# alibaba/TorchEasyRec

Hardware: NVIDIA H100
Metric: samples/sec (DLRM-Criteo synth, train step fwd+bwd+optimizer) (higher is better)
Workload: dtype f32

## Files before the change

### torcheasyrec_b200/csrc/tzk_interact_wide.cu

```cuda
#include <stdint.h>
#include <stdio.h>
#include <stdlib.h>

#ifdef TZK_CPU_SHIM
#include "cuda_cpu_shim.h"
#include "sm90_cpu_emu.h"
#include "sm90_wgmma_emu.h"
typedef void* tzk_stream_t;
#define TZK_REQUIRE(cond, ...) do { if (!(cond)) return 1; } while (0)
#define TZK_CHECK_LAUNCH(name) do {} while (0)
#else
#include <cuda.h>
#include "tzk_common.cuh"
#define TZK_DYN_SMEM(type, name) extern __shared__ __align__(1024) type name[]
#include "tzk_launch.cuh"
#endif

namespace {
#ifndef TZK_CPU_SHIM
#include "tzk_sm90_ptx.h"
#endif
#include "tzk_tma.h"
#include "tzk_wgmma.cuh"
namespace tzk_itc {
__device__ __forceinline__ uint32_t cvt_tf32(float x) { return tf32_bits(x); }
__device__ __forceinline__ void mma_tf32(float (&c)[4], const uint32_t (&a)[4], const uint32_t (&b)[2]) { ::mma_tf32(c, a, b); }
}
#include "tzk_interact_tc.cuh"

__device__ __forceinline__ float4 load_l2(const float* p) {
#ifdef TZK_CPU_SHIM
  return *reinterpret_cast<const float4*>(p);
#else
  return __ldcg(reinterpret_cast<const float4*>(p));
#endif
}

constexpr int FB_M = 64;
constexpr int FB_THREADS = 512;
constexpr int FB_WARPS = FB_THREADS / 32;
constexpr int FB_CHUNKS = (tzk_itc::kRow + 31) / 32;
constexpr int FB_PAIR_CHUNKS = tzk_itc::kInter / 32;
constexpr int FB_BOX = 32 * 128;
constexpr int FB_STAGE = 4 * FB_BOX;
constexpr int FB_STAGES = 3;
constexpr int FB_LDP = 360;
constexpr int FB_P_OFF = FB_STAGES * FB_STAGE;
constexpr int FB_S_OFF = FB_P_OFF + FB_M * FB_LDP * 4;
constexpr int FB_IJ_OFF = FB_S_OFF + FB_WARPS * 32 * tzk_itc::kSS * 4;
constexpr int FB_BAR_OFF = FB_IJ_OFF + tzk_itc::kInter * 2;
constexpr int FB_SMEM = FB_BAR_OFF + FB_STAGES * 8;

struct FbParams {
  const float* dz; int64_t ld_dz;
  const float* dense; int64_t ld_dense;
  const float* sparse; int64_t ld_sparse;
  float* d_dense; int64_t ld_ddense;
  float* d_sparse; int64_t ld_dsparse;
  int64_t M;
};

__global__ void __launch_bounds__(FB_THREADS, 1)
interact_wide_bwd_kernel(const __grid_constant__ CUtensorMap map_whi, const __grid_constant__ CUtensorMap map_wlo,
                         FbParams p) {
  TZK_DYN_SMEM(uint8_t, smem);
  float* P = reinterpret_cast<float*>(smem + FB_P_OFF);
  uint64_t* full = reinterpret_cast<uint64_t*>(smem + FB_BAR_OFF);
  const int warp = threadIdx.x >> 5, lane = threadIdx.x & 31, g = lane >> 2, t = lane & 3;
  const int64_t m0 = (int64_t)blockIdx.x * FB_M;

  if (threadIdx.x == 0) {
    for (int s = 0; s < FB_STAGES; ++s) mbar_init(full + s, 1);
    fence_mbarrier_init();
  }
  float* S = reinterpret_cast<float*>(smem + FB_S_OFF) + warp * (32 * tzk_itc::kSS);
  unsigned short* pair_ij = reinterpret_cast<unsigned short*>(smem + FB_IJ_OFF);
  tzk_itc::init_pair_ij(pair_ij);
  for (int i = lane; i < 32 * tzk_itc::kSS; i += 32) S[i] = 0.f;
  __syncthreads();
  auto col_chunk = [](int c) { return (c + FB_PAIR_CHUNKS) % FB_CHUNKS; };
  auto load = [&](int c) {
    uint8_t* sb = smem + (c % FB_STAGES) * FB_STAGE;
    uint64_t* bar = full + c % FB_STAGES;
    const int n0 = col_chunk(c) * 32;
    mbar_expect_tx(bar, FB_STAGE);
    tma_load_2d(sb, &map_whi, bar, 0, n0);
    tma_load_2d(sb + FB_BOX, &map_whi, bar, 32, n0);
    tma_load_2d(sb + 2 * FB_BOX, &map_wlo, bar, 0, n0);
    tma_load_2d(sb + 3 * FB_BOX, &map_wlo, bar, 32, n0);
  };
  if (threadIdx.x == 0)
    for (int c = 0; c < FB_STAGES; ++c) load(c);

  const int wm = warp & 3, wn = warp >> 2;
  const int r = wm * 16 + g;
  uint32_t ah[8][4], al[8][4];
#pragma unroll
  for (int kk = 0; kk < 8; ++kk) {
    const int k0 = kk * 8 + t, k1 = k0 + 4;
    const int64_t ra = m0 + r, rb = ra + 8;
    const float a[4] = {ra < p.M ? __ldg(p.dz + ra * p.ld_dz + k0) : 0.f, rb < p.M ? __ldg(p.dz + rb * p.ld_dz + k0) : 0.f,
                        ra < p.M ? __ldg(p.dz + ra * p.ld_dz + k1) : 0.f, rb < p.M ? __ldg(p.dz + rb * p.ld_dz + k1) : 0.f};
#pragma unroll
    for (int i = 0; i < 4; ++i) {
      ah[kk][i] = tf32_bits(a[i]);
      al[kk][i] = tf32_bits(a[i] - __uint_as_float(ah[kk][i]));
    }
  }
  const int n = wn * 8 + g;
  for (int c = 0; c < FB_CHUNKS; ++c) {
    const int s = c % FB_STAGES;
    mbar_wait(full + s, (uint32_t)(c / FB_STAGES) & 1u);
    const uint32_t* whi = reinterpret_cast<const uint32_t*>(smem + s * FB_STAGE);
    const uint32_t* wlo = whi + 2 * FB_BOX / 4;
    float acc[4] = {0.f, 0.f, 0.f, 0.f};
#pragma unroll
    for (int kk = 0; kk < 8; ++kk) {
      const uint32_t* bh_box = whi + (kk >> 2) * (FB_BOX / 4);
      const uint32_t* bl_box = wlo + (kk >> 2) * (FB_BOX / 4);
      const int k0 = (kk & 3) * 8 + t, k1 = k0 + 4;
      const uint32_t bh[2] = {bh_box[swz(n, k0)], bh_box[swz(n, k1)]};
      const uint32_t bl[2] = {bl_box[swz(n, k0)], bl_box[swz(n, k1)]};
      float part[4] = {0.f, 0.f, 0.f, 0.f};
      mma_tf32(part, al[kk], bh);
      mma_tf32(part, ah[kk], bl);
      mma_tf32(part, ah[kk], bh);
#pragma unroll
      for (int q = 0; q < 4; ++q) acc[q] += part[q];
    }
    const int col = col_chunk(c) * 32 + wn * 8 + 2 * t;
    if (col < tzk_itc::kInter) {
      *reinterpret_cast<float2*>(P + r * FB_LDP + col) = make_float2(acc[0], acc[1]);
      *reinterpret_cast<float2*>(P + (r + 8) * FB_LDP + col) = make_float2(acc[2], acc[3]);
    } else if (col < tzk_itc::kRow) {
      const int e = col - tzk_itc::kInter;
#pragma unroll
      for (int h = 0; h < 2; ++h) {
        const int64_t row = m0 + r + 8 * h;
        if (row >= p.M) continue;
        float* dst = e < tzk_itc::kD ? p.d_dense + row * p.ld_ddense + e : p.d_sparse + row * p.ld_dsparse + (e - tzk_itc::kD);
        *reinterpret_cast<float2*>(dst) = make_float2(acc[2 * h], acc[2 * h + 1]);
      }
    }
    __syncthreads();
    if (threadIdx.x == 0 && c + FB_STAGES < FB_CHUNKS) load(c + FB_STAGES);
  }

  for (int i = warp; i < FB_M; i += FB_WARPS) {
    const int64_t b = m0 + i;
    if (b >= p.M) break;
    float* dd = p.d_dense + b * p.ld_ddense;
    float* ds = p.d_sparse + b * p.ld_dsparse;
    float4 pass[4];
#pragma unroll
    for (int q = 0; q < 4; ++q) {
      const int row = g + 8 * q;
      pass[q] = row == 0 ? load_l2(dd + 4 * t)
              : row < tzk_itc::kN ? load_l2(ds + (row - 1) * tzk_itc::kD + 4 * t)
              : make_float4(0.f, 0.f, 0.f, 0.f);
    }
    tzk_itc::bwd_sample(P + i * FB_LDP, p.dense + b * p.ld_dense, p.sparse + b * p.ld_sparse, pass, pair_ij, S, dd, ds,
                        lane);
  }
}

constexpr int FF_M = 128;
constexpr int FF_THREADS = 256;
constexpr int FF_WARPS = FF_THREADS / 32;
constexpr int FF_X_BYTES = FF_M * 128;
constexpr int FF_W_BYTES = 64 * 128;
constexpr int FF_STAGE = FF_X_BYTES + 2 * FF_W_BYTES;
constexpr int FF_STAGES = 3;
constexpr int FF_E_OFF = FF_STAGES * FF_STAGE;
constexpr int FF_BAR_OFF = FF_E_OFF + FF_X_BYTES;
constexpr int FF_SMEM = FF_BAR_OFF + FF_STAGES * 8;
static_assert(FF_WARPS * tzk_itc::kInter * 4 <= FF_X_BYTES, "staging rows overflow their region");
constexpr int FF_SPARSE0 = tzk_itc::kInter + tzk_itc::kD;

struct FfParams {
  const float* dense; int64_t ld_dense;
  const float* sparse; int64_t ld_sparse;
  float* pairs; int64_t ld_pairs;
  const float* bias;
  float* y; int64_t ld_y;
  int64_t M;
};

__device__ __forceinline__ void fence_proxy_async() {
#ifndef TZK_CPU_SHIM
  asm volatile("fence.proxy.async;" ::: "memory");
#endif
}

__global__ void __launch_bounds__(FF_THREADS, 2)
interact_wide_fwd_kernel(const __grid_constant__ CUtensorMap map_pairs, const __grid_constant__ CUtensorMap map_dense,
                         const __grid_constant__ CUtensorMap map_sparse, const __grid_constant__ CUtensorMap map_whi, const __grid_constant__ CUtensorMap map_wlo,
                         FfParams p) {
  TZK_DYN_SMEM(uint8_t, smem);
  uint64_t* full = reinterpret_cast<uint64_t*>(smem + FF_BAR_OFF);
  const int warp = threadIdx.x >> 5, lane = threadIdx.x & 31, g = lane >> 2, t = lane & 3;
  const int64_t m0 = (int64_t)blockIdx.x * FF_M;
  const int64_t m_end = p.M - m0 < FF_M ? p.M : m0 + FF_M;

  if (threadIdx.x == 0) {
    for (int s = 0; s < FF_STAGES; ++s) mbar_init(full + s, 1);
    fence_mbarrier_init();
  }
  {
    float* O = reinterpret_cast<float*>(smem + FF_E_OFF) + warp * tzk_itc::kInter;
    if (lane == 0) O[tzk_itc::kP] = 0.f;
    int rowbase[4];
    tzk_itc::pair_rowbase(g, rowbase);
    int64_t b = m0 + warp;
    float4 x[4];
    if (b < m_end) {
#pragma unroll
      for (int j = 0; j < 4; ++j) x[j] = tzk_itc::load_x4(p.dense + b * p.ld_dense, p.sparse + b * p.ld_sparse, g + 8 * j, 4 * t);
    }
    for (; b < m_end; b += FF_WARPS) {
      float4 xn[4];
      const int64_t bn = b + FF_WARPS;
      if (bn < m_end) {
#pragma unroll
        for (int j = 0; j < 4; ++j)
          xn[j] = tzk_itc::load_x4(p.dense + bn * p.ld_dense, p.sparse + bn * p.ld_sparse, g + 8 * j, 4 * t);
      }
      tzk_itc::fwd_sample(x, rowbase, O, p.pairs + b * p.ld_pairs, lane);
      if (bn < m_end) {
#pragma unroll
        for (int j = 0; j < 4; ++j) x[j] = xn[j];
      }
    }
  }
  fence_proxy_async();
  __syncthreads();

  auto load = [&](int c) {
    uint8_t* sb = smem + (c % FF_STAGES) * FF_STAGE;
    uint64_t* bar = full + c % FF_STAGES;
    mbar_expect_tx(bar, c == FB_PAIR_CHUNKS ? FF_STAGE + FF_X_BYTES : FF_STAGE);
    if (c < FB_PAIR_CHUNKS) {
      tma_load_2d(sb, &map_pairs, bar, 32 * c, (int)m0);
    } else if (c == FB_PAIR_CHUNKS) {
      tma_load_2d(sb, &map_dense, bar, 0, (int)m0);
      tma_load_2d(smem + FF_E_OFF, &map_sparse, bar, 0, (int)m0);
    } else {
      tma_load_2d(sb, &map_sparse, bar, 32 * c - FF_SPARSE0, (int)m0);
    }
    tma_load_2d(sb + FF_X_BYTES, &map_whi, bar, 32 * c, 0);
    tma_load_2d(sb + FF_X_BYTES + FF_W_BYTES, &map_wlo, bar, 32 * c, 0);
  };
  if (threadIdx.x == 0)
    for (int c = 0; c < FF_STAGES; ++c) load(c);

  const int r = warp * 16 + g;
  float acc[32], part[32];
#pragma unroll
  for (int i = 0; i < 32; ++i) acc[i] = 0.f;
  for (int c = 0; c < FB_CHUNKS; ++c) {
    const int s = c % FF_STAGES;
    mbar_wait(full + s, (uint32_t)(c / FF_STAGES) & 1u);
    const float* xs = reinterpret_cast<const float*>(smem + s * FF_STAGE);
    const uint8_t* whi = smem + s * FF_STAGE + FF_X_BYTES;
    const uint8_t* wlo = whi + FF_W_BYTES;
#pragma unroll
    for (int ks = 0; ks < 4; ++ks) {
      const int k0 = ks * 8 + t, k1 = k0 + 4;
      const bool sp = ks >= 2 && c == FB_PAIR_CHUNKS;
      const float* as = sp ? reinterpret_cast<const float*>(smem + FF_E_OFF) : xs;
      const int x16 = sp ? 16 : 0;
      const float a[4] = {as[swz(r, k0) ^ x16], as[swz(r + 8, k0) ^ x16], as[swz(r, k1) ^ x16], as[swz(r + 8, k1) ^ x16]};
      uint32_t ah[4], al[4];
#pragma unroll
      for (int i = 0; i < 4; ++i) {
        ah[i] = tf32_bits(a[i]);
        al[i] = tf32_bits(a[i] - __uint_as_float(ah[i]));
      }
      wgmma_fence();
      wgmma_3xtf32<64>(part, ah, al, wgmma_desc(whi, ks), wgmma_desc(wlo, ks));
      wgmma_commit();
      wgmma_wait<0>();
#pragma unroll
      for (int i = 0; i < 32; ++i) {
        wgmma_reg_fence(part[i]);
        acc[i] += part[i];
      }
    }
    __syncthreads();
    if (threadIdx.x == 0 && c + FF_STAGES < FB_CHUNKS) load(c + FF_STAGES);
  }
#pragma unroll
  for (int nt = 0; nt < 8; ++nt) {
    const int col = nt * 8 + 2 * t;
    const float b0 = p.bias ? __ldg(p.bias + col) : 0.f, b1 = p.bias ? __ldg(p.bias + col + 1) : 0.f;
#pragma unroll
    for (int h = 0; h < 2; ++h) {
      const int64_t row = m0 + r + 8 * h;
      if (row >= p.M) continue;
      float2 o = make_float2(acc[4 * nt + 2 * h] + b0, acc[4 * nt + 2 * h + 1] + b1);
      o.x = fmaxf(o.x, 0.f);
      o.y = fmaxf(o.y, 0.f);
      *reinterpret_cast<float2*>(p.y + row * p.ld_y + col) = o;
    }
  }
}

__global__ void split_w_kernel(const float* __restrict__ w, int64_t ld_w, int K, float* __restrict__ hi,
                               float* __restrict__ lo) {
  const int i = blockIdx.x * blockDim.x + threadIdx.x;
  if (i < K * 64) {
    const float v = w[(int64_t)(i / K) * ld_w + i % K];
    const float h = tf32_rna(v);
    hi[i] = h;
    lo[i] = tf32_rna(v - h);
  }
}

#include "tzk_wgrad3x.cuh"

constexpr int WW_ZT = 64 * 128;

__global__ void __launch_bounds__(WG_THREADS, 2)
interact_wide_wgrad_kernel(const __grid_constant__ CUtensorMap map_x0, const __grid_constant__ CUtensorMap map_x1,
                           const __grid_constant__ CUtensorMap map_x2, const __grid_constant__ CUtensorMap map_dz,
                           WgParams p) {
  TZK_DYN_SMEM(uint8_t, smem);
  uint8_t* zt = smem + WG_STAGES * WG_STAGE;
  uint64_t* full = reinterpret_cast<uint64_t*>(zt + 2 * WW_ZT);
  int* boxes = reinterpret_cast<int*>(full + WG_STAGES);

  const int warp = threadIdx.x >> 5, lane = threadIdx.x & 31, g = lane >> 2, t = lane & 3;
  const int jt = blockIdx.x % p.k_tiles;
  const int64_t slab = blockIdx.x / p.k_tiles;
  const int64_t row0 = slab * p.slab_rows;
  const int64_t rows = (p.M - row0 < p.slab_rows) ? p.M - row0 : p.slab_rows;
  const int num_c = (int)((rows + WG_ROWS - 1) / WG_ROWS);

  if (threadIdx.x == 0) {
    for (int s = 0; s < WG_STAGES; ++s) mbar_init(full + s, 1);
    fence_mbarrier_init();
    for (int b = 0; b < 4; ++b) {
      const int box = jt * 4 + b, s = wg_source(p.src, box);
      boxes[b] = s;
      boxes[4 + b] = wg_pick(p.src.col0, s) + 32 * (box - wg_pick(p.src.first, s));
    }
  }
  __syncthreads();
  auto load = [&](int c) {
    uint8_t* sb = smem + (c % WG_STAGES) * WG_STAGE;
    uint64_t* bar = full + c % WG_STAGES;
    const int r = (int)(row0 + (int64_t)c * WG_ROWS);
    mbar_expect_tx(bar, WG_A + WG_B);
#pragma unroll 1
    for (int b = 0; b < 4; ++b) {
      const int s = *reinterpret_cast<volatile int*>(boxes + b), col = *reinterpret_cast<volatile int*>(boxes + 4 + b);
      tma_load_2d(sb + b * WG_BOX, s == 0 ? &map_x0 : s == 1 ? &map_x1 : &map_x2, bar, col, r);
    }
#pragma unroll
    for (int b = 0; b < 2; ++b) tma_load_2d(sb + WG_A + b * WG_BOX, &map_dz, bar, b * 32, r);
  };
  if (threadIdx.x == 0)
    for (int c = 0; c < WG_STAGES && c < num_c; ++c) load(c);

  const int xc = (warp >> 2) * 64 + (warp & 3) * 16 + g;
  const int tn = threadIdx.x & 63, tq = threadIdx.x >> 6;
  uint32_t* zhi = reinterpret_cast<uint32_t*>(zt);
  uint32_t* zlo = zhi + WW_ZT / 4;
  float acc[32], part[32];
#pragma unroll
  for (int i = 0; i < 32; ++i) acc[i] = 0.f;
  for (int c = 0; c < num_c; ++c) {
    const int s = c % WG_STAGES;
    mbar_wait(full + s, (uint32_t)(c / WG_STAGES) & 1u);
    const float* xs = reinterpret_cast<const float*>(smem + s * WG_STAGE);
    const float* zs = reinterpret_cast<const float*>(smem + s * WG_STAGE + WG_A);
    auto at = [](const float* base, int m, int col) { return base[(col >> 5) * (WG_BOX / 4) + swz(m, col & 31)]; };
#pragma unroll
    for (int h = 0; h < 2; ++h) {
      const int m = 4 * tq + 16 * h;
      float hi[4], lo[4];
#pragma unroll
      for (int j = 0; j < 4; ++j) {
        const float v = at(zs, m + j, tn);
        hi[j] = tf32_rna(v);
        lo[j] = tf32_rna(v - hi[j]);
      }
      *reinterpret_cast<float4*>(zhi + swz(tn, m)) = make_float4(hi[0], hi[1], hi[2], hi[3]);
      *reinterpret_cast<float4*>(zlo + swz(tn, m)) = make_float4(lo[0], lo[1], lo[2], lo[3]);
    }
    fence_proxy_async();
    __syncthreads();
#pragma unroll
    for (int ks = 0; ks < WG_ROWS / 8; ++ks) {
      const int m = ks * 8 + t;
      const float a[4] = {at(xs, m, xc), at(xs, m, xc + 8), at(xs, m + 4, xc), at(xs, m + 4, xc + 8)};
      uint32_t ah[4], al[4];
#pragma unroll
      for (int i = 0; i < 4; ++i) {
        ah[i] = tf32_bits(a[i]);
        al[i] = tf32_bits(a[i] - __uint_as_float(ah[i]));
      }
      wgmma_fence();
      wgmma_tf32<64>(part, ah, wgmma_desc(zlo, ks), false);
      wgmma_tf32<64>(part, al, wgmma_desc(zhi, ks), true);
      wgmma_tf32<64>(part, ah, wgmma_desc(zhi, ks), true);
      wgmma_commit();
      wgmma_wait<0>();
#pragma unroll
      for (int i = 0; i < 32; ++i) {
        wgmma_reg_fence(part[i]);
        acc[i] += part[i];
      }
    }
    __syncthreads();
    if (threadIdx.x == 0 && c + WG_STAGES < num_c) load(c + WG_STAGES);
  }
  float* out = p.partial + ((int64_t)slab * p.k_tiles + jt) * 128 * 64;
#pragma unroll
  for (int i = 0; i < 8; ++i)
#pragma unroll
    for (int h = 0; h < 2; ++h)
      *reinterpret_cast<float2*>(out + (int64_t)(xc + 8 * h) * 64 + 8 * i + 2 * t) =
          make_float2(acc[4 * i + 2 * h], acc[4 * i + 2 * h + 1]);
}

__global__ void split_wt_kernel(const float* __restrict__ w, int64_t ld_w, int K, float* __restrict__ hi,
                                float* __restrict__ lo) {
  const int i = blockIdx.x * blockDim.x + threadIdx.x;
  if (i < K * 64) {
    const int k = i >> 6, o = i & 63;
    const float v = w[(int64_t)o * ld_w + k];
    const float h = tf32_rna(v);
    hi[i] = h;
    lo[i] = tf32_rna(v - h);
  }
}

}

extern "C" int tzk_interact_wide_bwd(const float* dz, int64_t ld_dz, const float* w, int64_t ld_w, const float* dense,
                                     int64_t ld_dense, const float* sparse, int64_t ld_sparse, int64_t M, float* d_dense,
                                     int64_t ld_ddense, float* d_sparse, int64_t ld_dsparse, float* wt_hi, float* wt_lo,
                                     tzk_stream_t stream) {
  TZK_REQUIRE(M > 0, "interact_wide_bwd: M must be positive");
  TZK_REQUIRE(ld_w >= tzk_itc::kRow, "interact_wide_bwd: w needs %d columns", tzk_itc::kRow);
  const int64_t lds[] = {ld_dz, ld_w, ld_dense, ld_sparse, ld_ddense, ld_dsparse};
  for (int64_t ld : lds) TZK_REQUIRE(ld % 4 == 0, "interact_wide_bwd: row strides must be multiples of 4 floats");
  const void* ptrs[] = {dz, w, dense, sparse, d_dense, d_sparse, wt_hi, wt_lo};
  for (const void* q : ptrs)
    TZK_REQUIRE(q && reinterpret_cast<uintptr_t>(q) % 16 == 0, "interact_wide_bwd: NULL or not 16-B aligned pointer");
  cudaStream_t st = reinterpret_cast<cudaStream_t>(stream);
  TZK_LAUNCH((split_wt_kernel), (tzk_itc::kRow * 64 + 255) / 256, 256, 0, st, w, ld_w, tzk_itc::kRow, wt_hi, wt_lo);
  CUtensorMap mh, ml;
  TZK_REQUIRE(!make_map(&mh, wt_hi, tzk_itc::kRow, 64, 64, 32) && !make_map(&ml, wt_lo, tzk_itc::kRow, 64, 64, 32),
              "interact_wide_bwd: tensor-map encoding failed");
  FbParams p;
  p.dz = dz; p.ld_dz = ld_dz; p.dense = dense; p.ld_dense = ld_dense; p.sparse = sparse; p.ld_sparse = ld_sparse;
  p.d_dense = d_dense; p.ld_ddense = ld_ddense; p.d_sparse = d_sparse; p.ld_dsparse = ld_dsparse; p.M = M;
#ifndef TZK_CPU_SHIM
  static bool configured = false;
  if (!configured) {
    cudaFuncSetAttribute(interact_wide_bwd_kernel, cudaFuncAttributeMaxDynamicSharedMemorySize, FB_SMEM);
    configured = true;
  }
#endif
  TZK_LAUNCH((interact_wide_bwd_kernel), (unsigned)((M + FB_M - 1) / FB_M), FB_THREADS, FB_SMEM, st, mh, ml, p);
  TZK_CHECK_LAUNCH("interact_wide_bwd_kernel");
  return 0;
}

extern "C" int tzk_interact_wide_fwd(const float* dense, int64_t ld_dense, const float* sparse, int64_t ld_sparse,
                                     const float* w, int64_t ld_w, const float* bias, int64_t M, float* y, int64_t ld_y,
                                     float* pairs, int64_t ld_pairs, float* w_hi, float* w_lo, tzk_stream_t stream) {
  TZK_REQUIRE(M > 0, "interact_wide_fwd: M must be positive");
  TZK_REQUIRE(ld_w >= tzk_itc::kRow && ld_y >= 64 && ld_pairs >= tzk_itc::kInter && ld_dense >= tzk_itc::kD &&
              ld_sparse >= tzk_itc::kRow - FF_SPARSE0, "interact_wide_fwd: row stride shorter than the row");
  const int64_t lds[] = {ld_dense, ld_sparse, ld_w, ld_y, ld_pairs};
  for (int64_t ld : lds) TZK_REQUIRE(ld % 4 == 0, "interact_wide_fwd: row strides must be multiples of 4 floats");
  const void* ptrs[] = {dense, sparse, w, y, pairs, w_hi, w_lo};
  for (const void* q : ptrs)
    TZK_REQUIRE(q && reinterpret_cast<uintptr_t>(q) % 16 == 0, "interact_wide_fwd: NULL or not 16-B aligned pointer");
  cudaStream_t st = reinterpret_cast<cudaStream_t>(stream);
  TZK_LAUNCH((split_w_kernel), (tzk_itc::kRow * 64 + 255) / 256, 256, 0, st, w, ld_w, tzk_itc::kRow, w_hi, w_lo);
  CUtensorMap mp, md, ms, mh, ml;
  TZK_REQUIRE(!make_map(&mp, pairs, M, tzk_itc::kInter, ld_pairs, FF_M) &&
              !make_map(&md, dense, M, tzk_itc::kD, ld_dense, FF_M) &&
              !make_map(&ms, sparse, M, tzk_itc::kRow - FF_SPARSE0, ld_sparse, FF_M) &&
              !make_map(&mh, w_hi, 64, tzk_itc::kRow, tzk_itc::kRow, 64) &&
              !make_map(&ml, w_lo, 64, tzk_itc::kRow, tzk_itc::kRow, 64), "interact_wide_fwd: tensor-map encoding failed");
  FfParams p;
  p.dense = dense; p.ld_dense = ld_dense; p.sparse = sparse; p.ld_sparse = ld_sparse; p.pairs = pairs;
  p.ld_pairs = ld_pairs; p.bias = bias; p.y = y; p.ld_y = ld_y; p.M = M;
#ifndef TZK_CPU_SHIM
  static bool configured = false;
  if (!configured) {
    cudaFuncSetAttribute(interact_wide_fwd_kernel, cudaFuncAttributeMaxDynamicSharedMemorySize, FF_SMEM);
    configured = true;
  }
#endif
  TZK_LAUNCH((interact_wide_fwd_kernel), (unsigned)((M + FF_M - 1) / FF_M), FF_THREADS, FF_SMEM, st, mp, md, ms, mh, ml, p);
  TZK_CHECK_LAUNCH("interact_wide_fwd_kernel");
  return 0;
}

extern "C" int tzk_interact_wide_wgrad(const float* dz, int64_t ld_dz, const float* pairs, int64_t ld_pairs,
                                       const float* dense, int64_t ld_dense, const float* sparse, int64_t ld_sparse,
                                       int64_t M, int32_t slabs, float* partial, float* dw, int64_t ld_dw,
                                       tzk_stream_t stream) {
  TZK_REQUIRE(M > 0 && slabs > 0, "interact_wide_wgrad: M and slabs must be positive");
  TZK_REQUIRE(ld_dw >= tzk_itc::kRow, "interact_wide_wgrad: dw needs %d columns", tzk_itc::kRow);
  const int64_t lds[] = {ld_dz, ld_pairs, ld_dense, ld_sparse};
  for (int64_t ld : lds) TZK_REQUIRE(ld % 4 == 0, "interact_wide_wgrad: row strides must be multiples of 4 floats");
  const void* ptrs[] = {dz, pairs, dense, sparse, partial, dw};
  for (const void* q : ptrs)
    TZK_REQUIRE(q && reinterpret_cast<uintptr_t>(q) % 16 == 0, "interact_wide_wgrad: NULL or not 16-B aligned pointer");
  CUtensorMap mx[WG_SRC], mz;
  TZK_REQUIRE(!make_map(&mx[0], pairs, M, tzk_itc::kInter, ld_pairs, WG_ROWS) &&
              !make_map(&mx[1], sparse, M, tzk_itc::kRow - FF_SPARSE0, ld_sparse, WG_ROWS) &&
              !make_map(&mx[2], dense, M, tzk_itc::kD, ld_dense, WG_ROWS) &&
              !make_map(&mz, dz, M, 64, ld_dz, WG_ROWS), "interact_wide_wgrad: tensor-map encoding failed");
  const WgSources src = {{0, FB_PAIR_CHUNKS, FB_CHUNKS - 1, FB_CHUNKS}, {0, 0, 0}, {0, FF_SPARSE0, tzk_itc::kInter},
                         {tzk_itc::kInter, tzk_itc::kRow - FF_SPARSE0, tzk_itc::kD}};
  TZK_REQUIRE(wgrad3x_launch<interact_wide_wgrad_kernel>(mx, mz, src, M, slabs, partial, dw, ld_dw,
                                                         reinterpret_cast<cudaStream_t>(stream), 2 * WW_ZT) == 0,
              "interact_wide_wgrad: launch failed");
  return 0;
}
```

### torcheasyrec_b200/csrc/tzk_sm90_ptx.h

```cpp

__device__ __forceinline__ uint32_t smem_u32(const void* p) { return (uint32_t)__cvta_generic_to_shared(p); }

__device__ __forceinline__ void mbar_init(uint64_t* bar, uint32_t count) {
  asm volatile("mbarrier.init.shared::cta.b64 [%0], %1;" ::"r"(smem_u32(bar)), "r"(count));
}
__device__ __forceinline__ void mbar_expect_tx(uint64_t* bar, uint32_t bytes) {
  asm volatile("mbarrier.arrive.expect_tx.shared::cta.b64 _, [%0], %1;" ::"r"(smem_u32(bar)), "r"(bytes) : "memory");
}
__device__ __forceinline__ void mbar_wait(uint64_t* bar, uint32_t parity) {
  asm volatile(
      "{\n\t.reg .pred p;\n\t"
      "WAIT_LOOP:\n\t"
      "mbarrier.try_wait.parity.shared::cta.b64 p, [%0], %1;\n\t"
      "@p bra DONE;\n\t"
      "bra WAIT_LOOP;\n\t"
      "DONE:\n\t}" ::"r"(smem_u32(bar)), "r"(parity)
      : "memory");
}
__device__ __forceinline__ void fence_mbarrier_init() { asm volatile("fence.mbarrier_init.release.cluster;" ::: "memory"); }

__device__ __forceinline__ void tma_load_2d(void* dst, const CUtensorMap* map, uint64_t* bar, int c0, int c1) {
  asm volatile(
      "cp.async.bulk.tensor.2d.shared::cluster.global.mbarrier::complete_tx::bytes [%0], [%1, {%3, %4}], [%2];"
      ::"r"(smem_u32(dst)), "l"(map), "r"(smem_u32(bar)), "r"(c0), "r"(c1)
      : "memory");
}

__device__ __forceinline__ uint32_t tf32_bits(float x) {
  uint32_t r;
  asm("cvt.rna.tf32.f32 %0, %1;" : "=r"(r) : "f"(x));
  return r;
}
__device__ __forceinline__ float tf32_rna(float x) { return __uint_as_float(tf32_bits(x)); }
__device__ __forceinline__ void mma_tf32(float (&c)[4], const uint32_t (&a)[4], const uint32_t (&b)[2]) {
  asm volatile("mma.sync.aligned.m16n8k8.row.col.f32.tf32.tf32.f32 {%0,%1,%2,%3}, {%4,%5,%6,%7}, {%8,%9}, {%0,%1,%2,%3};"
               : "+f"(c[0]), "+f"(c[1]), "+f"(c[2]), "+f"(c[3])
               : "r"(a[0]), "r"(a[1]), "r"(a[2]), "r"(a[3]), "r"(b[0]), "r"(b[1]));
}
```

### torcheasyrec_b200/csrc/tzk_wgmma.cuh

```cuda
#pragma once

__device__ __forceinline__ uint64_t wgmma_desc(const void* box, int ks) {
  const uint32_t a = smem_u32(box) + 32u * (uint32_t)ks;
  return (uint64_t)((a >> 4) & 0x3fffu) | (1ull << 16) | ((uint64_t)(1024 >> 4) << 32) | (1ull << 62);
}

#ifndef TZK_CPU_SHIM
__device__ __forceinline__ void wgmma_fence() { asm volatile("wgmma.fence.sync.aligned;" ::: "memory"); }
__device__ __forceinline__ void wgmma_commit() { asm volatile("wgmma.commit_group.sync.aligned;" ::: "memory"); }
template <int N>
__device__ __forceinline__ void wgmma_wait() { asm volatile("wgmma.wait_group.sync.aligned %0;" ::"n"(N) : "memory"); }
__device__ __forceinline__ void wgmma_reg_fence(float& r) { asm volatile("" : "+f"(r)::"memory"); }

template <int N>
__device__ __forceinline__ void wgmma_tf32(float (&d)[N / 2], const uint32_t (&a)[4], uint64_t desc, bool scale_d);

template <>
__device__ __forceinline__ void wgmma_tf32<64>(float (&d)[32], const uint32_t (&a)[4], uint64_t desc, bool scale_d) {
  asm volatile(
      "{\n\t.reg .pred p;\n\tsetp.ne.b32 p, %37, 0;\n\t"
      "wgmma.mma_async.sync.aligned.m64n64k8.f32.tf32.tf32 "
      "{%0,%1,%2,%3,%4,%5,%6,%7,%8,%9,%10,%11,%12,%13,%14,%15,"
      "%16,%17,%18,%19,%20,%21,%22,%23,%24,%25,%26,%27,%28,%29,%30,%31}, {%32,%33,%34,%35}, %36, p, 1, 1;\n\t}"
      : "+f"(d[0]), "+f"(d[1]), "+f"(d[2]), "+f"(d[3]), "+f"(d[4]), "+f"(d[5]), "+f"(d[6]), "+f"(d[7]),
        "+f"(d[8]), "+f"(d[9]), "+f"(d[10]), "+f"(d[11]), "+f"(d[12]), "+f"(d[13]), "+f"(d[14]), "+f"(d[15]),
        "+f"(d[16]), "+f"(d[17]), "+f"(d[18]), "+f"(d[19]), "+f"(d[20]), "+f"(d[21]), "+f"(d[22]), "+f"(d[23]),
        "+f"(d[24]), "+f"(d[25]), "+f"(d[26]), "+f"(d[27]), "+f"(d[28]), "+f"(d[29]), "+f"(d[30]), "+f"(d[31])
      : "r"(a[0]), "r"(a[1]), "r"(a[2]), "r"(a[3]), "l"(desc), "r"((int)scale_d));
}
#endif

template <int N>
__device__ __forceinline__ void wgmma_3xtf32(float (&part)[N / 2], const uint32_t (&ah)[4], const uint32_t (&al)[4],
                                             uint64_t hi_b, uint64_t lo_b) {
  wgmma_tf32<N>(part, al, hi_b, false);
  wgmma_tf32<N>(part, ah, lo_b, true);
  wgmma_tf32<N>(part, ah, hi_b, true);
}
```

Baseline: 50.95 million.

## Make interaction backward persistent with TMA-fed dZ and per-warpgroup wgmma pipeline

The backward interaction kernel becomes persistent: the grid is capped at the SM count and each CTA loops over 64-row tiles. dZ is now fetched by TMA into a ring of four stages with full/empty mbarriers, which lets the next tile's loads overlap the current tile's epilogue. The per-warp mma.sync 3xTF32 GEMM is replaced by per-warpgroup m64n32k8 wgmma, with each of the four warpgroups owning one stage's column chunk. This adds complex producer/consumer barrier logic, and the wgmma calls wait synchronously after every step, which limits how much latency they can hide. Optional globaltimer stamps are included for profiling.

```diff
diff --git a/torcheasyrec_b200/csrc/tzk_interact_wide.cu b/torcheasyrec_b200/csrc/tzk_interact_wide.cu
--- a/torcheasyrec_b200/csrc/tzk_interact_wide.cu
+++ b/torcheasyrec_b200/csrc/tzk_interact_wide.cu
@@ -7,6 +7,7 @@
 #include "sm90_cpu_emu.h"
 #include "sm90_wgmma_emu.h"
 typedef void* tzk_stream_t;
+inline void mbar_arrive(uint64_t* bar) { mbar_expect_tx(bar, 0); }
 #define TZK_REQUIRE(cond, ...) do { if (!(cond)) return 1; } while (0)
 #define TZK_CHECK_LAUNCH(name) do {} while (0)
 #else
@@ -41,18 +42,36 @@
 constexpr int FB_WARPS = FB_THREADS / 32;
 constexpr int FB_CHUNKS = (tzk_itc::kRow + 31) / 32;
 constexpr int FB_PAIR_CHUNKS = tzk_itc::kInter / 32;
+constexpr int FB_ITEMS = 1 + FB_CHUNKS;
 constexpr int FB_BOX = 32 * 128;
-constexpr int FB_STAGE = 4 * FB_BOX;
-constexpr int FB_STAGES = 3;
+constexpr int FB_HALF = 2 * FB_BOX;
+constexpr int FB_STAGE = 2 * FB_HALF;
+constexpr int FB_STAGES = 4;
 constexpr int FB_LDP = 360;
 constexpr int FB_P_OFF = FB_STAGES * FB_STAGE;
 constexpr int FB_S_OFF = FB_P_OFF + FB_M * FB_LDP * 4;
 constexpr int FB_IJ_OFF = FB_S_OFF + FB_WARPS * 32 * tzk_itc::kSS * 4;
 constexpr int FB_BAR_OFF = FB_IJ_OFF + tzk_itc::kInter * 2;
-constexpr int FB_SMEM = FB_BAR_OFF + FB_STAGES * 8;
+constexpr int FB_SMEM = FB_BAR_OFF + 4 * FB_STAGES * 8;
+static_assert(FB_HALF == FB_M * 128, "a dZ box [64 x 32 floats] fills half a stage");
+static_assert(FB_STAGES == 4, "stage i % 4 is read by warpgroup i % 4");
+static_assert(FB_SMEM <= 227 * 1024, "over the opt-in shared memory of one CTA");
+
+#ifdef TZK_FB_TIMING
+__device__ unsigned long long* fb_timing;
+__device__ __forceinline__ unsigned long long fb_now() {
+  unsigned long long t;
+  asm volatile("mov.u64 %0, %%globaltimer;" : "=l"(t));
+  return t;
+}
+#define FB_STAMP(tile, slot) do { if (threadIdx.x == 0) fb_timing[4 * (tile) + (slot)] = fb_now(); } while (0)
+#define FB_STAMP_LAST(tile, slot) do { if ((threadIdx.x & 31) == 0) atomicMax(fb_timing + 4 * (tile) + (slot), fb_now()); } while (0)
+#else
+#define FB_STAMP(tile, slot) do {} while (0)
+#define FB_STAMP_LAST(tile, slot) do {} while (0)
+#endif
 
 struct FbParams {
-  const float* dz; int64_t ld_dz;
   const float* dense; int64_t ld_dense;
   const float* sparse; int64_t ld_sparse;
   float* d_dense; int64_t ld_ddense;
@@ -61,16 +80,21 @@
 };
 
 __global__ void __launch_bounds__(FB_THREADS, 1)
-interact_wide_bwd_kernel(const __grid_constant__ CUtensorMap map_whi, const __grid_constant__ CUtensorMap map_wlo,
-                         FbParams p) {
+interact_wide_bwd_kernel(const __grid_constant__ CUtensorMap map_dz, const __grid_constant__ CUtensorMap map_whi,
+                         const __grid_constant__ CUtensorMap map_wlo, FbParams p) {
   TZK_DYN_SMEM(uint8_t, smem);
   float* P = reinterpret_cast<float*>(smem + FB_P_OFF);
   uint64_t* full = reinterpret_cast<uint64_t*>(smem + FB_BAR_OFF);
+  uint64_t* empty = full + 2 * FB_STAGES;
   const int warp = threadIdx.x >> 5, lane = threadIdx.x & 31, g = lane >> 2, t = lane & 3;
-  const int64_t m0 = (int64_t)blockIdx.x * FB_M;
+  const int wg = warp >> 2, r = (warp & 3) * 16 + g;
+  const int64_t tiles = (p.M + FB_M - 1) / FB_M;
 
   if (threadIdx.x == 0) {
-    for (int s = 0; s < FB_STAGES; ++s) mbar_init(full + s, 1);
+    for (int s = 0; s < 2 * FB_STAGES; ++s) {
+      mbar_init(full + s, 1);
+      mbar_init(empty + s, 4);
+    }
     fence_mbarrier_init();
   }
   float* S = reinterpret_cast<float*>(smem + FB_S_OFF) + warp * (32 * tzk_itc::kSS);
@@ -78,89 +102,127 @@
   tzk_itc::init_pair_ij(pair_ij);
   for (int i = lane; i < 32 * tzk_itc::kSS; i += 32) S[i] = 0.f;
   __syncthreads();
-  auto col_chunk = [](int c) { return (c + FB_PAIR_CHUNKS) % FB_CHUNKS; };
-  auto load = [&](int c) {
-    uint8_t* sb = smem + (c % FB_STAGES) * FB_STAGE;
-    uint64_t* bar = full + c % FB_STAGES;
-    const int n0 = col_chunk(c) * 32;
-    mbar_expect_tx(bar, FB_STAGE);
-    tma_load_2d(sb, &map_whi, bar, 0, n0);
-    tma_load_2d(sb + FB_BOX, &map_whi, bar, 32, n0);
-    tma_load_2d(sb + 2 * FB_BOX, &map_wlo, bar, 0, n0);
-    tma_load_2d(sb + 3 * FB_BOX, &map_wlo, bar, 32, n0);
+  auto load = [&](int64_t item, int h) {
+    const int64_t tile = blockIdx.x + item / FB_ITEMS * gridDim.x;
+    if (tile >= tiles) return;
+    if (item >= FB_STAGES) mbar_wait(empty + 2 * (item % FB_STAGES) + h, (uint32_t)(item / FB_STAGES - 1) & 1u);
+    const int j = (int)(item % FB_ITEMS);
+    uint8_t* hb = smem + (item % FB_STAGES) * FB_STAGE + h * FB_HALF;
+    uint64_t* bar = full + 2 * (item % FB_STAGES) + h;
+    mbar_expect_tx(bar, FB_HALF);
+    if (j == 0) {
+      tma_load_2d(hb, &map_dz, bar, 32 * h, (int)(tile * FB_M));
+    } else {
+      tma_load_2d(hb, &map_whi, bar, 32 * h, (j - 1) * 32);
+      tma_load_2d(hb + FB_BOX, &map_wlo, bar, 32 * h, (j - 1) * 32);
+    }
   };
   if (threadIdx.x == 0)
-    for (int c = 0; c < FB_STAGES; ++c) load(c);
-
-  const int wm = warp & 3, wn = warp >> 2;
-  const int r = wm * 16 + g;
-  uint32_t ah[8][4], al[8][4];
-#pragma unroll
-  for (int kk = 0; kk < 8; ++kk) {
-    const int k0 = kk * 8 + t, k1 = k0 + 4;
-    const int64_t ra = m0 + r, rb = ra + 8;
-    const float a[4] = {ra < p.M ? __ldg(p.dz + ra * p.ld_dz + k0) : 0.f, rb < p.M ? __ldg(p.dz + rb * p.ld_dz + k0) : 0.f,
-                        ra < p.M ? __ldg(p.dz + ra * p.ld_dz + k1) : 0.f, rb < p.M ? __ldg(p.dz + rb * p.ld_dz + k1) : 0.f};
-#pragma unroll
-    for (int i = 0; i < 4; ++i) {
-      ah[kk][i] = tf32_bits(a[i]);
-      al[kk][i] = tf32_bits(a[i] - __uint_as_float(ah[kk][i]));
-    }
-  }
-  const int n = wn * 8 + g;
-  for (int c = 0; c < FB_CHUNKS; ++c) {
-    const int s = c % FB_STAGES;
-    mbar_wait(full + s, (uint32_t)(c / FB_STAGES) & 1u);
-    const uint32_t* whi = reinterpret_cast<const uint32_t*>(smem + s * FB_STAGE);
-    const uint32_t* wlo = whi + 2 * FB_BOX / 4;
-    float acc[4] = {0.f, 0.f, 0.f, 0.f};
-#pragma unroll
-    for (int kk = 0; kk < 8; ++kk) {
-      const uint32_t* bh_box = whi + (kk >> 2) * (FB_BOX / 4);
-      const uint32_t* bl_box = wlo + (kk >> 2) * (FB_BOX / 4);
-      const int k0 = (kk & 3) * 8 + t, k1 = k0 + 4;
-      const uint32_t bh[2] = {bh_box[swz(n, k0)], bh_box[swz(n, k1)]};
-      const uint32_t bl[2] = {bl_box[swz(n, k0)], bl_box[swz(n, k1)]};
-      float part[4] = {0.f, 0.f, 0.f, 0.f};
-      mma_tf32(part, al[kk], bh);
-      mma_tf32(part, ah[kk], bl);
-      mma_tf32(part, ah[kk], bh);
-#pragma unroll
-      for (int q = 0; q < 4; ++q) acc[q] += part[q];
-    }
-    const int col = col_chunk(c) * 32 + wn * 8 + 2 * t;
-    if (col < tzk_itc::kInter) {
-      *reinterpret_cast<float2*>(P + r * FB_LDP + col) = make_float2(acc[0], acc[1]);
-      *reinterpret_cast<float2*>(P + (r + 8) * FB_LDP + col) = make_float2(acc[2], acc[3]);
-    } else if (col < tzk_itc::kRow) {
-      const int e = col - tzk_itc::kInter;
-#pragma unroll
-      for (int h = 0; h < 2; ++h) {
-        const int64_t row = m0 + r + 8 * h;
-        if (row >= p.M) continue;
-        float* dst = e < tzk_itc::kD ? p.d_dense + row * p.ld_ddense + e : p.d_sparse + row * p.ld_dsparse + (e - tzk_itc::kD);
-        *reinterpret_cast<float2*>(dst) = make_float2(acc[2 * h], acc[2 * h + 1]);
+    for (int i = 0; i < FB_STAGES; ++i) {
+      load(i, 0);
+      load(i, 1);
+    }
+
+  int64_t item0 = 0;
+  for (int64_t tile = blockIdx.x; tile < tiles; tile += gridDim.x, item0 += FB_ITEMS) {
+    const int64_t m0 = tile * FB_M;
+    FB_STAMP(tile, 0);
+    float a[8][4];
+    {
+      const int s = (int)(item0 % FB_STAGES);
+      mbar_wait(full + 2 * s, (uint32_t)(item0 / FB_STAGES) & 1u);
+      mbar_wait(full + 2 * s + 1, (uint32_t)(item0 / FB_STAGES) & 1u);
+      const float* zs = reinterpret_cast<const float*>(smem + s * FB_STAGE);
+#pragma unroll
+      for (int kk = 0; kk < 8; ++kk) {
+        const float* box = zs + (kk >> 2) * (FB_HALF / 4);
+        const int k0 = (kk & 3) * 8 + t, k1 = k0 + 4;
+        a[kk][0] = box[swz(r, k0)];
+        a[kk][1] = box[swz(r + 8, k0)];
+        a[kk][2] = box[swz(r, k1)];
+        a[kk][3] = box[swz(r + 8, k1)];
       }
     }
     __syncthreads();
-    if (threadIdx.x == 0 && c + FB_STAGES < FB_CHUNKS) load(c + FB_STAGES);
-  }
-
-  for (int i = warp; i < FB_M; i += FB_WARPS) {
-    const int64_t b = m0 + i;
-    if (b >= p.M) break;
-    float* dd = p.d_dense + b * p.ld_ddense;
-    float* ds = p.d_sparse + b * p.ld_dsparse;
-    float4 pass[4];
-#pragma unroll
-    for (int q = 0; q < 4; ++q) {
-      const int row = g + 8 * q;
-      pass[q] = row == 0 ? load_l2(dd + 4 * t)
-              : row < tzk_itc::kN ? load_l2(ds + (row - 1) * tzk_itc::kD + 4 * t)
-              : make_float4(0.f, 0.f, 0.f, 0.f);
-    }
-    tzk_itc::bwd_sample(P + i * FB_LDP, p.dense + b * p.ld_dense, p.sparse + b * p.ld_sparse, pass, pair_ij, S, dd, ds,
-                        lane);
+    if (warp < 4 && lane == 0) {
+      mbar_arrive(empty + 2 * (item0 % FB_STAGES));
+      mbar_arrive(empty + 2 * (item0 % FB_STAGES) + 1);
+    }
+    if (threadIdx.x == 0) {
+      load(item0 + FB_STAGES, 0);
+      load(item0 + FB_STAGES, 1);
+    }
+    FB_STAMP(tile, 1);
+
+    for (int c = (int)((wg - item0 - 1) & 3); c < FB_CHUNKS; c += 4) {
+      const int64_t item = item0 + 1 + c;
+      float acc[16], part[16];
+#pragma unroll
+      for (int i = 0; i < 16; ++i) acc[i] = 0.f;
+#pragma unroll
+      for (int kk = 0; kk < 8; ++kk) {
+        const int h = kk >> 2;
+        const uint8_t* whi = smem + wg * FB_STAGE + h * FB_HALF;
+        if ((kk & 3) == 0) mbar_wait(full + 2 * wg + h, (uint32_t)(item / FB_STAGES) & 1u);
+        uint32_t ah[4], al[4];
+#pragma unroll
+        for (int i = 0; i < 4; ++i) {
+          ah[i] = tf32_bits(a[kk][i]);
+          al[i] = tf32_bits(a[kk][i] - __uint_as_float(ah[i]));
+        }
+        wgmma_fence();
+        wgmma_3xtf32<32>(part, ah, al, wgmma_desc(whi, kk & 3), wgmma_desc(whi + FB_BOX, kk & 3));
+        wgmma_commit();
+        wgmma_wait<0>();
+#pragma unroll
+        for (int i = 0; i < 16; ++i) {
+          wgmma_reg_fence(part[i]);
+          acc[i] += part[i];
+        }
+        if ((kk & 3) == 3) {
+          __syncwarp();
+          if (lane == 0) mbar_arrive(empty + 2 * wg + h);
+          if ((threadIdx.x & 127) == 0) load(item + FB_STAGES, h);
+        }
+      }
+#pragma unroll
+      for (int i = 0; i < 4; ++i) {
+        const int col = c * 32 + i * 8 + 2 * t;
+        if (col < tzk_itc::kInter) {
+          *reinterpret_cast<float2*>(P + r * FB_LDP + col) = make_float2(acc[4 * i], acc[4 * i + 1]);
+          *reinterpret_cast<float2*>(P + (r + 8) * FB_LDP + col) = make_float2(acc[4 * i + 2], acc[4 * i + 3]);
+        } else if (col < tzk_itc::kRow) {
+          const int e = col - tzk_itc::kInter;
+#pragma unroll
+          for (int h = 0; h < 2; ++h) {
+            const int64_t row = m0 + r + 8 * h;
+            if (row >= p.M) continue;
+            float* dst = e < tzk_itc::kD ? p.d_dense + row * p.ld_ddense + e : p.d_sparse + row * p.ld_dsparse + (e - tzk_itc::kD);
+            *reinterpret_cast<float2*>(dst) = make_float2(acc[4 * i + 2 * h], acc[4 * i + 2 * h + 1]);
+          }
+        }
+      }
+    }
+    __syncthreads();
+    FB_STAMP(tile, 2);
+
+    for (int i = warp; i < FB_M; i += FB_WARPS) {
+      const int64_t b = m0 + i;
+      if (b >= p.M) break;
+      float* dd = p.d_dense + b * p.ld_ddense;
+      float* ds = p.d_sparse + b * p.ld_dsparse;
+      float4 pass[4];
+#pragma unroll
+      for (int q = 0; q < 4; ++q) {
+        const int row = g + 8 * q;
+        pass[q] = row == 0 ? load_l2(dd + 4 * t)
+                : row < tzk_itc::kN ? load_l2(ds + (row - 1) * tzk_itc::kD + 4 * t)
+                : make_float4(0.f, 0.f, 0.f, 0.f);
+      }
+      tzk_itc::bwd_sample(P + i * FB_LDP, p.dense + b * p.ld_dense, p.sparse + b * p.ld_sparse, pass, pair_ij, S, dd, ds,
+                          lane);
+    }
+    FB_STAMP_LAST(tile, 3);
   }
 }
 
@@ -438,6 +500,12 @@
 
 }
 
+#ifdef TZK_FB_TIMING
+extern "C" int tzk_interact_wide_bwd_timing(unsigned long long* buf) {
+  return cudaMemcpyToSymbol(fb_timing, &buf, sizeof(buf)) == cudaSuccess ? 0 : 1;
+}
+#endif
+
 extern "C" int tzk_interact_wide_bwd(const float* dz, int64_t ld_dz, const float* w, int64_t ld_w, const float* dense,
                                      int64_t ld_dense, const float* sparse, int64_t ld_sparse, int64_t M, float* d_dense,
                                      int64_t ld_ddense, float* d_sparse, int64_t ld_dsparse, float* wt_hi, float* wt_lo,
@@ -449,13 +517,20 @@
   const void* ptrs[] = {dz, w, dense, sparse, d_dense, d_sparse, wt_hi, wt_lo};
   for (const void* q : ptrs)
     TZK_REQUIRE(q && reinterpret_cast<uintptr_t>(q) % 16 == 0, "interact_wide_bwd: NULL or not 16-B aligned pointer");
+  int dev = 0, sms = 0;
+  TZK_REQUIRE(cudaGetDevice(&dev) == cudaSuccess &&
+              cudaDeviceGetAttribute(&sms, cudaDevAttrMultiProcessorCount, dev) == cudaSuccess && sms > 0,
+              "interact_wide_bwd: no device");
+#ifdef TZK_CPU_SHIM
+  if (const char* e = getenv("TZK_EMU_SMS")) sms = atoi(e);
+#endif
   cudaStream_t st = reinterpret_cast<cudaStream_t>(stream);
   TZK_LAUNCH((split_wt_kernel), (tzk_itc::kRow * 64 + 255) / 256, 256, 0, st, w, ld_w, tzk_itc::kRow, wt_hi, wt_lo);
-  CUtensorMap mh, ml;
-  TZK_REQUIRE(!make_map(&mh, wt_hi, tzk_itc::kRow, 64, 64, 32) && !make_map(&ml, wt_lo, tzk_itc::kRow, 64, 64, 32),
-              "interact_wide_bwd: tensor-map encoding failed");
+  CUtensorMap mz, mh, ml;
+  TZK_REQUIRE(!make_map(&mz, dz, M, 64, ld_dz, FB_M) && !make_map(&mh, wt_hi, tzk_itc::kRow, 64, 64, 32) &&
+              !make_map(&ml, wt_lo, tzk_itc::kRow, 64, 64, 32), "interact_wide_bwd: tensor-map encoding failed");
   FbParams p;
-  p.dz = dz; p.ld_dz = ld_dz; p.dense = dense; p.ld_dense = ld_dense; p.sparse = sparse; p.ld_sparse = ld_sparse;
+  p.dense = dense; p.ld_dense = ld_dense; p.sparse = sparse; p.ld_sparse = ld_sparse;
   p.d_dense = d_dense; p.ld_ddense = ld_ddense; p.d_sparse = d_sparse; p.ld_dsparse = ld_dsparse; p.M = M;
 #ifndef TZK_CPU_SHIM
   static bool configured = false;
@@ -464,7 +539,8 @@
     configured = true;
   }
 #endif
-  TZK_LAUNCH((interact_wide_bwd_kernel), (unsigned)((M + FB_M - 1) / FB_M), FB_THREADS, FB_SMEM, st, mh, ml, p);
+  const int64_t tiles = (M + FB_M - 1) / FB_M;
+  TZK_LAUNCH((interact_wide_bwd_kernel), (unsigned)(tiles < sms ? tiles : sms), FB_THREADS, FB_SMEM, st, mz, mh, ml, p);
   TZK_CHECK_LAUNCH("interact_wide_bwd_kernel");
   return 0;
 }
diff --git a/torcheasyrec_b200/csrc/tzk_sm90_ptx.h b/torcheasyrec_b200/csrc/tzk_sm90_ptx.h
--- a/torcheasyrec_b200/csrc/tzk_sm90_ptx.h
+++ b/torcheasyrec_b200/csrc/tzk_sm90_ptx.h
@@ -6,6 +6,9 @@
 }
 __device__ __forceinline__ void mbar_expect_tx(uint64_t* bar, uint32_t bytes) {
   asm volatile("mbarrier.arrive.expect_tx.shared::cta.b64 _, [%0], %1;" ::"r"(smem_u32(bar)), "r"(bytes) : "memory");
+}
+__device__ __forceinline__ void mbar_arrive(uint64_t* bar) {
+  asm volatile("mbarrier.arrive.shared::cta.b64 _, [%0];" ::"r"(smem_u32(bar)) : "memory");
 }
 __device__ __forceinline__ void mbar_wait(uint64_t* bar, uint32_t parity) {
   asm volatile(
diff --git a/torcheasyrec_b200/csrc/tzk_wgmma.cuh b/torcheasyrec_b200/csrc/tzk_wgmma.cuh
--- a/torcheasyrec_b200/csrc/tzk_wgmma.cuh
+++ b/torcheasyrec_b200/csrc/tzk_wgmma.cuh
@@ -28,6 +28,17 @@
         "+f"(d[24]), "+f"(d[25]), "+f"(d[26]), "+f"(d[27]), "+f"(d[28]), "+f"(d[29]), "+f"(d[30]), "+f"(d[31])
       : "r"(a[0]), "r"(a[1]), "r"(a[2]), "r"(a[3]), "l"(desc), "r"((int)scale_d));
 }
+
+template <>
+__device__ __forceinline__ void wgmma_tf32<32>(float (&d)[16], const uint32_t (&a)[4], uint64_t desc, bool scale_d) {
+  asm volatile(
+      "{\n\t.reg .pred p;\n\tsetp.ne.b32 p, %21, 0;\n\t"
+      "wgmma.mma_async.sync.aligned.m64n32k8.f32.tf32.tf32 "
+      "{%0,%1,%2,%3,%4,%5,%6,%7,%8,%9,%10,%11,%12,%13,%14,%15}, {%16,%17,%18,%19}, %20, p, 1, 1;\n\t}"
+      : "+f"(d[0]), "+f"(d[1]), "+f"(d[2]), "+f"(d[3]), "+f"(d[4]), "+f"(d[5]), "+f"(d[6]), "+f"(d[7]),
+        "+f"(d[8]), "+f"(d[9]), "+f"(d[10]), "+f"(d[11]), "+f"(d[12]), "+f"(d[13]), "+f"(d[14]), "+f"(d[15])
+      : "r"(a[0]), "r"(a[1]), "r"(a[2]), "r"(a[3]), "l"(desc), "r"((int)scale_d));
+}
 #endif
 
 template <int N>
```

Measured after the change: 52.68 million (median of 6 runs). +3.4%, better.
